# 42jaylonw/shifu

Measured on AMD Instinct MI355X. Metric: env-steps/sec (whole node), A1 12-dof 4096 envs/GPU, higher is better.
Workload: dtype f32

## Files before the change

### include/shifu_amd.h

```cpp
#ifndef SHIFU_AMD_H
#define SHIFU_AMD_H

#include <stdint.h>

#ifdef __cplusplus
extern "C" {
#endif

#define SHF_ABI_VERSION 22

#define SHF_MAX_BODIES 32
#define SHF_MAX_DOFS 32
#define SHF_MAX_POINTS 176
#define SHF_MAX_BOXES 4
#define SHF_MAX_SPHERES 8
#define SHF_MAX_CAPSULES 16
#define SHF_MAX_PAIRS 96
#define SHF_MAX_SELF_CONTACTS 8
#define SHF_MAX_ABOX 16
#define SHF_MAX_HARD_CONTACTS 16
#define SHF_MAX_LINK_CONTACTS 16

#define SHF_MAX_HULLS 8
#define SHF_HULL_MAX_VERTS 32
// ... 176 lines not shown
};
#define SHF_CONTACT_HIST_BINS 26

enum {
  SHF_REFRESH_DOF = 1,
  SHF_REFRESH_ROOT = 2,
  SHF_REFRESH_BODY = 4,
  SHF_REFRESH_CONTACT = 8,
  SHF_REFRESH_JACOBIAN = 16,
  SHF_REFRESH_ALL = 31
};

typedef struct ShfSim ShfSim;

const char* shf_last_error(void);
int shf_abi_version(void);

int shf_sim_create(const ShfSimParams* params, ShfSim** out);
int shf_sim_destroy(ShfSim* sim);
int shf_sim_set_terrain(ShfSim* sim, const ShfTerrain* terrain);
int shf_sim_set_articulation(ShfSim* sim, const ShfModel* model);
int shf_model_bounds(ShfModel* model);
int shf_model_pgs_supported(const ShfModel* model, int32_t nboxes);
int shf_sim_set_hulls(ShfSim* sim, const ShfHullSet* hulls);
int shf_convex_manifold(int32_t n, const float* pairs_dev, const ShfHull* hull_a_dev_or_null, float offset, int32_t lanes,
                        float* out_dev, void* stream);
#define SHF_CAP_TEST_SLOTS 88
int shf_cap_select_test(int32_t n, const float* gaps_dev, const uint8_t* flags_dev, const int32_t* kmax_dev, uint8_t* kept_dev, void* stream);
int shf_sim_set_scene_flags(ShfSim* sim, int32_t flags);
int shf_sim_add_box(ShfSim* sim, const ShfBoxDesc* box);
int shf_sim_finalize(ShfSim* sim, int32_t num_envs, int64_t env_id_offset);
int shf_sim_layout(const ShfSim* sim, int32_t id, int64_t shape[4], int32_t* ndim, int32_t* dtype);
int shf_sim_bind(ShfSim* sim, int32_t id, void* device_ptr);
int shf_sim_reset_all(ShfSim* sim, const float* default_root_dev , const float* default_dof_dev ,
                      const float* env_origins_dev , void* stream);
int shf_sim_set_group(ShfSim* sim, int32_t lanes);
enum { SHF_MAP_BODY = 0, SHF_MAP_CHAIN = 1, SHF_MAP_CHAIN_SPLIT = 2 };
int shf_sim_set_mapping(ShfSim* sim, int32_t mapping);

int shf_sim_step(ShfSim* sim, void* stream);
typedef struct ShfLaunchPlan {
  const char* kernel;
  int32_t grid, block;
  int64_t lds_bytes;
} ShfLaunchPlan;
int shf_sim_step_plan(const ShfSim* sim, ShfLaunchPlan* plan);
// ... 362 lines not shown
```

### shifu_amd/_lib.py

```python
import ctypes as C
import os

from . import _abi

_HERE = os.path.dirname(os.path.abspath(__file__))
_PATH = os.environ.get("SHIFU_AMD_LIB") or os.path.join(_HERE, "libshifu_amd.so")
_lib = None

vp, i32, i64 = C.c_void_p, C.c_int32, C.c_int64
_SIGS = {
    "shf_abi_version": ([], i32),
    "shf_sim_create": ([C.POINTER(_abi.ShfSimParams), C.POINTER(vp)], i32),
    "shf_sim_destroy": ([vp], i32),
    "shf_sim_set_terrain": ([vp, C.POINTER(_abi.ShfTerrain)], i32),
    "shf_sim_set_articulation": ([vp, C.POINTER(_abi.ShfModel)], i32),
    "shf_model_bounds": ([C.POINTER(_abi.ShfModel)], i32),
    "shf_model_pgs_supported": ([C.POINTER(_abi.ShfModel), i32], i32),
    "shf_abb_step_pgs_is_wide": ([vp], i32),
    "shf_sim_add_box": ([vp, C.POINTER(_abi.ShfBoxDesc)], i32),
    "shf_sim_set_hulls": ([vp, C.POINTER(_abi.ShfHullSet)], i32),
    "shf_sim_set_scene_flags": ([vp, i32], i32),
    "shf_convex_manifold": ([i32, vp, vp, C.c_float, i32, vp, vp], i32),
    "shf_cap_select_test": ([i32, vp, vp, vp, vp, vp], i32),
    "shf_sim_finalize": ([vp, i32, i64], i32),
    "shf_sim_set_group": ([vp, i32], i32),
    "shf_sim_set_mapping": ([vp, i32], i32),
    "shf_sim_layout": ([vp, i32, C.POINTER(i64), C.POINTER(i32), C.POINTER(i32)], i32),
    "shf_sim_bind": ([vp, i32, vp], i32),
    "shf_sim_reset_all": ([vp, vp, vp, vp, vp], i32),
    "shf_sim_step": ([vp, vp], i32),
    "shf_sim_step_plan": ([vp, C.POINTER(_abi.ShfLaunchPlan)], i32),
    "shf_sim_refresh": ([vp, i32, vp], i32),
    "shf_sim_dynamics": ([vp, vp, vp, vp], i32),
    "shf_sim_floating_dynamics": ([vp, vp, vp, vp, vp], i32),
    "shf_sim_set_dof_command": ([vp, i32, vp, vp], i32),
    "shf_sim_set_pos_target_indexed": ([vp, vp, vp, i32, vp], i32),
    "shf_sim_apply_body_force": ([vp, vp, vp], i32),
    "shf_sim_apply_body_force_at_pos": ([vp, vp, vp, vp], i32),
    "shf_sim_commit_root_indexed": ([vp, vp, vp, i32, vp], i32),
    "shf_sim_commit_root_all": ([vp, vp, vp], i32),
# ... 106 lines not shown
```

### shifu_amd/csrc/shf_a1_chain.hip

```cpp
#include <hip/hip_runtime.h>

#include "shf_chain.h"
#include "shf_chain_hard.h"

template <int G, bool TW, bool SELF = false>
__global__ __launch_bounds__(256, (G == 32 ? 2 : 1)) void k_a1_chain(A1Args A) { a1_chain_step_body<G, A1Chain, TW, SELF>(A); }

#ifndef SHF_WR_FUSED
#define SHF_WR_FUSED 8
#endif
#ifndef SHF_WR_HOOK
#define SHF_WR_HOOK 0
#endif
template <bool TW, bool SELF>
__global__ __launch_bounds__(256, 2) void k_a1_chain_pgs(A1Args A) { a1_chain_step_body<32, A1Chain, TW, SELF, true, 8, false, SHF_WR_FUSED>(A); }
template <bool TW, bool SELF>
__global__ __launch_bounds__(256, 2) void k_a1_chain_pgs16(A1Args A) { a1_chain_step_body<32, A1Chain, TW, SELF, true, 16>(A); }
template <bool TW, bool SELF>
__global__ __launch_bounds__(256, 2) void k_a1_chain_tgs(A1Args A) { a1_chain_step_body<32, A1Chain, TW, SELF, true, 8, true, SHF_WR_FUSED>(A); }
template <bool TW, bool SELF>
__global__ __launch_bounds__(256, 2) void k_a1_chain_tgs16(A1Args A) { a1_chain_step_body<32, A1Chain, TW, SELF, true, 16, true>(A); }
#define SHF_PICK4(K, warped, self) ((self) ? ((warped) ? reinterpret_cast<const void*>(K<true, true>) : reinterpret_cast<const void*>(K<false, true>)) \
                                           : ((warped) ? reinterpret_cast<const void*>(K<true, false>) : reinterpret_cast<const void*>(K<false, false>)))
const void* shf_a1_chain_pgs_kernel(bool warped, bool self, bool k16, bool tgs) {
  if (tgs) return k16 ? SHF_PICK4(k_a1_chain_tgs16, warped, self) : SHF_PICK4(k_a1_chain_tgs, warped, self);
  return k16 ? SHF_PICK4(k_a1_chain_pgs16, warped, self) : SHF_PICK4(k_a1_chain_pgs, warped, self);
}
int shf_a1_chain_pgs_max_contacts(void) { return 16; }

template <bool TW, bool SELF, int KC, bool TGS>
DEV void sim_step_chain_pgs_body(const SimArgs& A) {
  extern __shared__ __attribute__((aligned(16))) float smem[];
  typedef A1Chain CD;
  constexpr int G = 32, nb = CD::NB, nd = CD::ND, NR = (CD::NEV + G - 1) / G;
  const int es = threadIdx.x / G, l = threadIdx.x % G;
  const int e = blockIdx.x * (256 / G) + es;
  stage_block<CHAIN_MODEL_BYTES>(A.model, smem);
  __syncthreads();
  const ShfModel* m = reinterpret_cast<const ShfModel*>(smem);
  if (e >= A.n) return;
  ChainLds L = chain_lds_carve<CD>(smem + CHAIN_MODEL_WORDS + es * chain_lds_words<CD>(0, SELF));
  const float* dof = A.dof + (size_t)e * nd * 2;
  const float* root = A.root + (size_t)e * 13;
  for (int i = l; i < 2 * nd; i += G) L.dofb[(i >> 1) * DOF_STRIDE + (i & 1)] = dof[i];
  if (l < 13) L.root[l] = root[l];
  GROUP_SYNC();
  StepCtx C;
  C.m = m; C.sp = A.sp; C.terr.t = A.terr; C.terr.h = A.heights; C.scene = nullptr;
  C.dropped = env_dropped(A.dropped, A.sp, e);
  C.mscale = A.mscale ? A.mscale + (size_t)e * nb : nullptr;
  const float mu = A.friction ? A.friction[e] : 1.0f;
// ... 6 lines not shown
  chain_substep_hard<G, CD, TW, SELF, KC, TGS, (KC == 8 ? SHF_WR_HOOK : 0)>(C, L, l, X, LP, RL, A.body_force ? A.body_force + (size_t)e * nb * 3 : nullptr, mu, L.xch);
  if (l < nd) {
    A.dof[((size_t)e * nd + l) * 2] = X.q;
    A.dof[((size_t)e * nd + l) * 2 + 1] = X.qd;
  }
  if (l < 13) A.root[(size_t)e * 13 + l] = L.root[l];
  for (int i = l; i < 3 * nb; i += G) A.contact[(size_t)e * nb * 3 + i] = L.xch[i];
}
template <bool TW, bool SELF>
__global__ __launch_bounds__(256, 2) void k_sim_step_chain_pgs(SimArgs A) { sim_step_chain_pgs_body<TW, SELF, 8, false>(A); }
template <bool TW, bool SELF>
__global__ __launch_bounds__(256, 2) void k_sim_step_chain_pgs16(SimArgs A) { sim_step_chain_pgs_body<TW, SELF, 16, false>(A); }
template <bool TW, bool SELF>
__global__ __launch_bounds__(256, 2) void k_sim_step_chain_tgs(SimArgs A) { sim_step_chain_pgs_body<TW, SELF, 8, true>(A); }
template <bool TW, bool SELF>
__global__ __launch_bounds__(256, 2) void k_sim_step_chain_tgs16(SimArgs A) { sim_step_chain_pgs_body<TW, SELF, 16, true>(A); }
const void* shf_sim_step_chain_pgs_kernel(bool warped, bool self, bool k16, bool tgs) {
  if (tgs) return k16 ? SHF_PICK4(k_sim_step_chain_tgs16, warped, self) : SHF_PICK4(k_sim_step_chain_tgs, warped, self);
  return k16 ? SHF_PICK4(k_sim_step_chain_pgs16, warped, self) : SHF_PICK4(k_sim_step_chain_pgs, warped, self);
}
size_t shf_sim_step_chain_pgs_lds_bytes(bool self) { return ((size_t)CHAIN_MODEL_WORDS + 8 * (size_t)chain_lds_words<A1Chain>(0, self)) * 4; }

bool shf_a1_chain_matches(const ShfModel& m) { return A1Chain::matches(m); }
size_t shf_a1_chain_lds_bytes(int G, int nobs, bool self) {
  const int epb = 256 / G;
  return ((size_t)CHAIN_MODEL_WORDS + TASK_WORDS + STATS_LDS_WORDS + (size_t)epb * chain_lds_words<A1Chain>(SCR_OBS + nobs, self)) * 4;
}
const void* shf_a1_chain_kernel(int G, bool warped, bool self) {
  if (self) {
    if (G != 32) return nullptr;
    return warped ? reinterpret_cast<const void*>(k_a1_chain<32, true, true>) : reinterpret_cast<const void*>(k_a1_chain<32, false, true>);
  }
  switch (G) {
    case 16: return warped ? reinterpret_cast<const void*>(k_a1_chain<16, true>) : reinterpret_cast<const void*>(k_a1_chain<16, false>);
    case 32: return warped ? reinterpret_cast<const void*>(k_a1_chain<32, true>) : reinterpret_cast<const void*>(k_a1_chain<32, false>);
    default: return nullptr;
  }
}
#ifdef SHF_PHASE_CLOCK
int shf_a1_chain_phase_cycles(unsigned long long* out, int n, int reset) {
  unsigned long long h[48];
  if (hipMemcpyFromSymbol(h, HIP_SYMBOL(g_phase_cycles), sizeof h) != hipSuccess) return 1;
  for (int k = 0; k < n && k < 48; k++) out[k] = h[k];
  if (reset) {
    unsigned long long z[48] = {};
    if (hipMemcpyToSymbol(HIP_SYMBOL(g_phase_cycles), z, sizeof z) != hipSuccess) return 1;
  }
  return 0;
}
// ... 10 lines not shown
```

### shifu_amd/csrc/shf_api.hip

```cpp
#include <hip/hip_runtime.h>
#include <dlfcn.h>

#include <cstdio>
#include <cstring>
#include <initializer_list>
#include <map>
#include <mutex>
#include <type_traits>
#include <utility>
#include <vector>
#include <algorithm>
#include <cmath>
#include <string>

#include "shf_device.h"
#include "shf_task.h"
#include "shf_arm.h"
#include "shf_dyn.h"

static thread_local std::string g_err;
static int fail(const std::string& msg) { g_err = msg; return 1; }
int shf_set_error(const std::string& msg) { return fail(msg); }
#define HIP_OK(call)                                                              \
  do {                                                                            \
// ... 11 lines not shown
  int32_t n = 0;
  int64_t env_off = 0;
  bool finalized = false;
  bool force_armed = false;
  bool force_at_pos = false;
  void* t[SHF_T_COUNT] = {};
  int group = 64;
  int mapping = SHF_MAP_BODY;
  int mapping_split = 0;
  int chain_group = 16;
  ShfHullSet hulls;
  bool has_hulls = false;
  int scene_flags = 0;
};

struct ShfA1Task {
  ShfSim* sim;
  ShfA1TaskParams tp;
  void* t[SHF_A1_COUNT] = {};
  int stats_ring = 256;
};

bool shf_a1_chain_matches(const ShfModel& m);
size_t shf_a1_chain_lds_bytes(int G, int nobs, bool self);
const void* shf_a1_chain_kernel(int G, bool warped, bool self);
const void* shf_a1_chain_pgs_kernel(bool warped, bool self, bool k16, bool tgs);
int shf_a1_chain_pgs_max_contacts(void);
const void* shf_sim_step_chain_pgs_kernel(bool warped, bool self, bool k16, bool tgs);
size_t shf_sim_step_chain_pgs_lds_bytes(bool self);
#ifdef SHF_PHASE_CLOCK
int shf_a1_chain_phase_cycles(unsigned long long* out, int n, int reset);
int shf_a1_chain_phase_waves(unsigned long long* out, int reset);
#endif

extern "C" const char* shf_last_error(void) { return g_err.c_str(); }
extern "C" int shf_abi_version(void) { return SHF_ABI_VERSION; }


#define SHF_DEFINE_SMALL_KERNELS
#ifdef SHF_UNITY
#define SHF_DEFINE_A1_KERNELS
#endif
#include "shf_kernels.h"
#ifndef SHF_UNITY
#define SHF_KERNEL(...) extern template __global__ void __VA_ARGS__;
#include "shf_kernel_list.h"
#undef SHF_KERNEL
// ... 274 lines not shown
  A.scene = (const ShfScene*)s->t[SHF_T_SCENE];
  A.nboxes = s->nboxes;
  A.n = s->n;
  A.dof = (float*)s->t[internal ? SHF_T_SIM_DOF : SHF_T_DOF_STATE];
  A.root = (float*)s->t[internal ? SHF_T_SIM_ROOT : SHF_T_ROOT_STATE];
  A.actors = 1 + s->nboxes;
  A.effort = (const float*)s->t[SHF_T_EFFORT];
  A.pos_tgt = (const float*)s->t[SHF_T_POS_TARGET];
  A.vel_tgt = (const float*)s->t[SHF_T_VEL_TARGET];
  A.body_force = nullptr;
  A.body_force_pos = nullptr;
  A.friction = (const float*)s->t[SHF_T_FRICTION];
  A.mscale = (const float*)s->t[SHF_T_BODY_MASS_SCALE];
  A.contact = (float*)s->t[internal ? SHF_T_SIM_CONTACT : SHF_T_CONTACT];
  A.dropped = (int32_t*)s->t[SHF_T_DROPPED];
  A.hulls = (s->model.nhull > 0 && s->model.link_collide != 0) ? (const ShfHullSet*)s->t[SHF_T_HULLS] : nullptr;
  if (s->t[SHF_T_CONTACT_HIST]) {
    A.dropped = (int32_t*)s->t[SHF_T_CONTACT_HIST];
    A.sp.max_contacts = (A.sp.max_contacts & 0xff) | SHF_HIST_FLAG;
  }
  return A;
}

static int lds_fits(size_t lds) {
  return lds > 160 * 1024 ? fail("kernel needs " + std::to_string(lds) + " B of LDS per block, the CU has 160 KiB") : 0;
}
static int grant_lds(const void* fn, size_t lds) {
  if (int r = lds_fits(lds)) return r;
  if (lds > 48 * 1024) {
    static std::mutex mu;
    static std::map<std::pair<int, const void*>, size_t> granted;
    int dev = 0;
    HIP_OK(hipGetDevice(&dev));
    std::lock_guard<std::mutex> lock(mu);
    size_t& have = granted[{dev, fn}];
    if (have < lds) {
      HIP_OK(hipFuncSetAttribute(fn, hipFuncAttributeMaxDynamicSharedMemorySize, (int)lds));
      have = lds;
    }
  }
  return 0;
}
template <typename K, typename... Args>
static int launch(K kernel, dim3 grid, dim3 block, size_t lds, void* stream, Args... args) {
  if (int r = grant_lds(reinterpret_cast<const void*>(kernel), lds)) return r;
  hipLaunchKernelGGL(kernel, grid, block, lds, (hipStream_t)stream, args...);
  HIP_OK(hipGetLastError());
  return 0;
// ... 345 lines not shown
  A.push = (float*)task->t[SHF_A1_PUSH]; A.origins = (float*)task->t[SHF_A1_ORIGINS];
  A.levels = (int64_t*)task->t[SHF_A1_LEVELS]; A.types = (const int64_t*)task->t[SHF_A1_TYPES];
  A.torigins = (const float*)task->t[SHF_A1_TORIGINS];
  A.reset_count = (int32_t*)task->t[SHF_A1_RESET_COUNT];
  A.done_sums = (float*)task->t[SHF_A1_DONE_SUMS];
  A.body_state = (float*)s->t[SHF_T_BODY_STATE];
  A.stats.acc = (unsigned long long*)task->t[SHF_A1_STATS_ACC];
  A.stats.out = (float*)task->t[SHF_A1_STATS];
  A.stats.ring = task->stats_ring;
  A.stats.out_cols = 16;
  return 0;
}

static int a1_step_plan(const ShfA1Task* task, Plan& P) {
  const ShfSim* s = task->sim;
  const int nobs = 12 + 2 * s->model.nd + s->model.nd * task->tp.num_history + task->tp.num_height_points;
  const int g = s->group, n = s->n;
  const bool self = sim_self(s), warped = s->terr.warped != 0;
  if (s->sp.solver != SHF_SOLVER_COMPLIANT) {
    if (s->mapping != SHF_MAP_CHAIN || s->chain_group != 32 || !shf_a1_chain_matches(s->model))
      return fail("shf_a1_step: ShfSimParams.solver = SHF_SOLVER_PGS runs on the chain mapping at 32 lanes per env (shf_sim_set_mapping)");
    if (s->sp.max_contacts > shf_a1_chain_pgs_max_contacts()) return fail("shf_a1_step: the fused A1 step's solve holds at most 16 constraints per env (ShfSimParams.max_contacts)");
    if (s->sp.pos_iters < 1) return fail("shf_a1_step: ShfSimParams.pos_iters must be >= 1 with SHF_SOLVER_PGS");
    return set_plan(P, shf_a1_chain_pgs_kernel(warped, self, s->sp.max_contacts > HCK, s->sp.solver == SHF_SOLVER_TGS), n, 8, 256, shf_a1_chain_lds_bytes(32, nobs, self));
  }
  if (s->mapping == SHF_MAP_CHAIN) {
    if (!shf_a1_chain_matches(s->model)) return fail("shf_a1_step: the articulation does not fit the chain mapping");
    const void* fn = shf_a1_chain_kernel(s->chain_group, warped, self);
    if (!fn) return fail(self ? "shf_a1_step: the chain mapping with self-collision runs at 32 lanes per env"
                              : "shf_a1_step: the chain mapping runs at 16 or 32 lanes per env");
    return set_plan(P, fn, n, 256 / s->chain_group, 256, shf_a1_chain_lds_bytes(s->chain_group, nobs, self));
  }
  if (warped && g == 64)
    return fail("shf_a1_step: a trimesh terrain needs 16 or 32 lanes per env (the 128-VGPR instantiation has no room for it)");
  if (self && g == 64) return fail("shf_a1_step: self-collision needs 16 or 32 lanes per env (no register room in the 128-VGPR instantiation)");
  const bool a1 = A1Dims::matches(s->model);
  if (a1 && g == 16) return fail("shf_a1_step: A1 has 17 bodies, the lane group must be 32 or 64");
  const void* fn;
  if (!a1) fn = self ? (g == 32 ? KFN(k_a1_step_self<32, DynDims>) : KFN(k_a1_step_self<16, DynDims>)) : PICK_LANES(g, k_a1_step, DynDims);
  else if (self) fn = warped ? KFN(k_a1_step_self<32, A1Dims>) : KFN(k_a1_step_self_a1_g32);
  else fn = g == 64 ? KFN(k_a1_step<64, A1Dims>) : warped ? KFN(k_a1_step<32, A1Dims>) : KFN(k_a1_step_a1_g32);
  return set_plan(P, fn, n, 256 / g, 256, sim_lds_bytes(s, g, TASK_WORDS + STATS_LDS_WORDS, SCR_OBS + nobs));
}
extern "C" int shf_a1_step_plan(const ShfA1Task* task, ShfLaunchPlan* out) {
  if (!task) return fail("shf_a1_step: null task");
  if (!out) return fail("shf_a1_step_plan: null argument");
  Plan P;
  return export_plan(a1_step_plan(task, P), P, out);
}
static int a1_step_launch(ShfA1Task* task, const float* raw_actions_dev, void* stream) {
  A1Args A;
  if (int r = a1_args(task, raw_actions_dev, "shf_a1_step", A)) return r;
  Plan P;
  if (int r = a1_step_plan(task, P)) return r;
// ... 200 lines not shown
```

### shifu_amd/csrc/shf_chain.h

```cpp
#pragma once
#include "shf_task.h"
#include "shf_link.h"

template <int NCH_, int NLK_, int NP_, int NEV_>
struct ChainDims {
  static constexpr int NCH = NCH_, NLK = NLK_, NB = 1 + NCH_ * (NLK_ + 1), ND = NCH_ * NLK_, NPC = NP_;
  static constexpr int NEV = NEV_;
  static constexpr int MAXPT = 9;
  static_assert(NEV_ >= NP_ && NEV_ <= 128, "evaluation slots: two 64-bit ballot words");
  DEV static constexpr int body(int c, int k) { return 1 + c * (NLK_ + 1) + k; }
  static bool matches(const ShfModel& m) {
    if (m.nb != NB || m.nd != ND || m.np != NPC || m.fixed_base || m.jtype[0] != SHF_JOINT_ROOT) return false;
    if (m.child_count[0] != NCH || m.nlevels != NLK) return false;
    if ((m.neval > 0 ? m.neval : m.np) != NEV) return false;
    int occupied = 0;
    for (int s = 0; s < NEV; s++) {
      const int i = m.pt_eval[s];
      if (i == -1) continue;
      if (i < 0 || i >= NPC || m.pt_slot[i] != s) return false;
      occupied++;
    }
    if (occupied != NPC) return false;
    for (int b = 0; b < NB; b++) {
      const int n = m.pt_count[b], i0 = m.pt_start[b];
// ... 23 lines not shown
};
typedef ChainDims<4, 3, 76, 88> A1Chain;

#define JREC_STRIDE 16
#define JREC_QD 9
#define JREC_T0 12
#define JREC_DE 13
#define JREC_S 0
#define JREC_C 6
#define CHAIN_MODEL_BYTES ((int)offsetof(ShfModel, link_collide))
#define CHAIN_MODEL_WORDS ((CHAIN_MODEL_BYTES / 4 + 3) & ~3)
static_assert(CHAIN_MODEL_BYTES % 16 == 0, "stage_block copies 16-byte words");
template <class CD>
__host__ __device__ inline int chain_lds_words(int min_tail, bool self = false) {
  int tail = (CD::NPC + (self ? SHF_MAX_SELF_CONTACTS : 0)) * PT_STRIDE;
  if (tail < min_tail) tail = min_tail;
  const int w = CD::NB * POSE_STRIDE + ((CD::NB * 6 + 3) & ~3) + (CD::ND + 1) * XCH_STRIDE + CD::ND * JREC_STRIDE +
                ((CD::ND * DOF_STRIDE + 3) & ~3) + root_words(1) + tail;
  return (w + 3) & ~3;
}
struct ChainLds : EnvLds {
  float* jrec;
  float* xroot;
};
template <class CD>
DEV ChainLds chain_lds_carve(float* base) {
  static_assert(CD::ND * XCH_STRIDE >= 3 * CD::NB, "the exchange slots double as the contact-force staging");
  ChainLds L;
  L.pose = base;
  L.acc = L.pose + CD::NB * POSE_STRIDE;
  L.xch = L.acc + ((CD::NB * 6 + 3) & ~3);
  L.xroot = L.xch + CD::ND * XCH_STRIDE;
  L.jrec = L.xroot + XCH_STRIDE;
  L.dofb = L.jrec + CD::ND * JREC_STRIDE;
  L.root = L.dofb + ((CD::ND * DOF_STRIDE + 3) & ~3);
  L.pt = L.root + root_words(1);
  return L;
}

DEV void chain_ext_force(const float* F, const float* com, const float* Rw, const float* p, float* pA) {
  if (F[0] == 0.0f && F[1] == 0.0f && F[2] == 0.0f) return;
  float cw[3], t[3];
  mv3(Rw, com, cw);
#pragma unroll
  for (int k = 0; k < 3; k++) cw[k] += p[k];
  cross3(cw, F, t);
// ... 43 lines not shown
    const int s = l + k * G;
    const int e = s < nev ? m->pt_eval[s] : -1;
    const int i = e < 0 ? 0 : e;
    P.idx[k] = e;
    P.body[k] = m->pt_body[i];
    P.rad[k] = m->pt_radius[i];
    P.thr[k] = (offset + P.rad[k]) * 1.01f + 1e-6f;
#pragma unroll
    for (int j = 0; j < 3; j++) P.pos[k][j] = m->pt_pos[i][j];
  }
}

DEV void terrain_height_gradient(const TerrainDev& T, float x, float y, float* h, float* gxo, float* gyo) {
  if (T.t.rows == 0) { *h = 0.0f; *gxo = 0.0f; *gyo = 0.0f; return; }
  float inv = 1.0f / T.t.hscale;
  float fx = (x + T.t.border) * inv, fy = (y + T.t.border) * inv;
  float fi = rclampf(floorf(fx), 0.0f, (float)(T.t.rows - 2)), fj = rclampf(floorf(fy), 0.0f, (float)(T.t.cols - 2));
  int i = (int)fi, j = (int)fj;
  float u = rclampf(fx - fi, 0.0f, 1.0f), v = rclampf(fy - fj, 0.0f, 1.0f);
  float vs = T.t.vscale;
  const int16_t* row0 = T.h + (size_t)i * T.t.cols + j;
  const int16_t* row1 = row0 + T.t.cols;
  float h00 = (float)row0[0] * vs, h10 = (float)row1[0] * vs, h01 = (float)row0[1] * vs, h11 = (float)row1[1] * vs;
  const bool lo = u + v <= 1.0f;
  float gx = (lo ? h10 : h11) - (lo ? h00 : h01);
  float gy = (lo ? h01 : h11) - (lo ? h00 : h10);
  *h = fmaf(lo ? v : 1.0f - v, lo ? gy : -gy, fmaf(lo ? u : 1.0f - u, lo ? gx : -gx, lo ? h00 : h11));
  *gxo = gx * inv; *gyo = gy * inv;
}
DEV void terrain_normal_from_gradient(const TerrainDev& T, float gx, float gy, float* n) {
  if (T.t.rows == 0) { n[0] = 0.0f; n[1] = 0.0f; n[2] = 1.0f; return; }
  const float nz = rsqrt_spec(fmaf(gy, gy, fmaf(gx, gx, 1.0f)));
  n[0] = -gx * nz; n[1] = -gy * nz; n[2] = nz;
}

struct SlotBits {
  unsigned long long w[2];
  DEV bool test(int s) const { return ((s < 64 ? w[0] >> s : w[1] >> (s - 64)) & 1ull) != 0ull; }
  DEV unsigned field(int s0, int n) const {
    const unsigned long long ww = s0 < 64 ? w[0] : w[1];
    return (unsigned)(ww >> (s0 & 63)) & ((1u << n) - 1u);
  }
};
template <int MAXPT>
struct SlotList {
  unsigned long long list;
// ... 521 lines not shown
  GROUP_SYNC();
  for (int b = l; b < NB; b += G) {
    const float* pb = L.pose + b * POSE_STRIDE;
    float Rw[9], pp[3], v[6], t[3], q[4];
#pragma unroll
    for (int k = 0; k < 9; k++) Rw[k] = pb[k];
#pragma unroll
    for (int k = 0; k < 3; k++) pp[k] = pb[9 + k];
#pragma unroll
    for (int k = 0; k < 6; k++) v[k] = pb[12 + k];
    float* o = stage + 13 * b;
#pragma unroll
    for (int k = 0; k < 3; k++) o[k] = L.root[k] + pp[k];
    mat_to_quat(Rw, q);
#pragma unroll
    for (int k = 0; k < 4; k++) o[3 + k] = q[k];
    cross3(v, pp, t);
#pragma unroll
    for (int k = 0; k < 3; k++) { o[7 + k] = v[3 + k] + t[k]; o[10 + k] = v[k]; }
  }
  GROUP_SYNC();
}

template <int G, class CD, bool TW, bool SELF, int KC, bool TGS, int WR>
DEV void chain_substep_hard(const StepCtx& C, const ChainLds& L, int l, DofLane& X, const ChainPoints<(CD::NEV + G - 1) / G>& P,
                            const RowLane& RL, const float* fext, float mu_shape, float* contact_out);
template <int G, class CD, bool TW, bool SELF = false, bool HARD = false, int KC = 8, bool TGS = false, int WR = 0>
DEV void a1_chain_step_body(const A1Args& A) {
  extern __shared__ __attribute__((aligned(16))) float smem[];
  constexpr int NLK = CD::NLK, nb = CD::NB, nd = CD::ND, NR = (CD::NEV + G - 1) / G;
  PHASE_BEGIN();
  float* stats_lds = smem + CHAIN_MODEL_WORDS + TASK_WORDS;
  stats_block_init(stats_lds);
  const int epb = 256 / G, es = threadIdx.x / G, l = threadIdx.x % G;
  const int e = blockIdx.x * epb + es;
  const int n = A.S.n;
  const unsigned long long stats_req = stats_step_request(A.stats);
  const uint64_t seed = A.tp->seed;
  __builtin_amdgcn_sched_barrier(0);
  constexpr int NW = (2 * nd + G - 1) / G;
  float pre_dof[NW], pre_root = 0.0f, pre_act = 0.0f;
#pragma unroll
  for (int k = 0; k < NW; k++) pre_dof[k] = 0.0f;
  static_assert(G >= 13 && G > nd, "one root word and one action per lane");
  const bool given = A.raw_actions != nullptr;
  if (e < n) {
#pragma unroll
    for (int k = 0; k < NW; k++)
      if (l + k * G < 2 * nd) pre_dof[k] = A.S.dof[(size_t)e * nd * 2 + l + k * G];
    if (l < 13) pre_root = A.S.root[(size_t)e * 13 + l];
    if (l < nd && given) pre_act = A.raw_actions[(size_t)e * nd + l];
  }
  StagedBlock<(int)sizeof(ShfA1TaskParams)> tp_words;
  StagedBlock<CHAIN_MODEL_BYTES> model_words;
  tp_words.load(A.tp);
  model_words.load(A.S.model);
  const unsigned long long stats_step = stats_step_take(stats_req);
  constexpr bool POSTFIX = !(HARD && !TGS);
  const unsigned stats_row_index = POSTFIX ? stats_slot(A.stats, stats_step) : 0u;
  if (e < n && l < nd && !given) pre_act = random_action(seed, A.env_off + e, stats_step, l);
#pragma unroll
  for (int k = 0; k < NW; k++) asm volatile("" : "+v"(pre_dof[k]));
  asm volatile("" : "+v"(pre_root), "+v"(pre_act));
  tp_words.pin();
  model_words.pin();
  tp_words.store(smem + CHAIN_MODEL_WORDS);
  model_words.store(smem);
  __syncthreads();
  PHASE_MARK(23);
  const ShfModel* m = reinterpret_cast<const ShfModel*>(smem);
  const ShfA1TaskParams& tp = *reinterpret_cast<const ShfA1TaskParams*>(smem + CHAIN_MODEL_WORDS);
  if (e >= n) return;
  const int H = tp.num_history, P = tp.num_height_points;
  const int nobs = 12 + 2 * nd + nd * H + P;
  const int env_words = chain_lds_words<CD>(SCR_OBS + nobs, SELF);
  ChainLds L = chain_lds_carve<CD>(smem + CHAIN_MODEL_WORDS + TASK_WORDS + STATS_LDS_WORDS + es * env_words);
  float* scr = L.pt;

#pragma unroll
  for (int k = 0; k < NW; k++) {
    const int i = l + k * G;
    if (i < 2 * nd) L.dofb[(i >> 1) * DOF_STRIDE + (i & 1)] = pre_dof[k];
  }
  if (l < 13) L.root[l] = pre_root;
  float act = 0.0f;
  if (l < nd) {
    act = rclampf(pre_act * tp.action_scale, -tp.clip_actions, tp.clip_actions);
    A.actions[(size_t)e * nd + l] = act;
  }
  GROUP_SYNC();

  if (l == 0) {
    const float gv[3] = {0.0f, 0.0f, -1.0f};
    float pg[3], blv[3], bav[3];
    quat_rotate_inverse(L.root + 3, L.root + 7, blv);
    quat_rotate_inverse(L.root + 3, L.root + 10, bav);
    quat_rotate_inverse(L.root + 3, gv, pg);
    float* o = A.base_vel + (size_t)e * 9;
#pragma unroll
    for (int k = 0; k < 3; k++) { o[k] = blv[k]; o[3 + k] = bav[k]; o[6 + k] = pg[k]; }
  }

  StepCtx C;
  C.m = m; C.sp = A.S.sp; C.terr.t = A.S.terr; C.terr.h = A.S.heights; C.scene = nullptr;
  if constexpr (HARD) C.dropped = env_dropped(A.S.dropped, A.S.sp, e);
  C.mscale = A.S.mscale ? A.S.mscale + (size_t)e * nb : nullptr;
  const float mu = A.S.friction[e];
  const int nsub = tp.decimation + (tp.extra_substep ? 1 : 0);
  const int dl = l < nd ? l : 0;
  DofLane X = {L.dofb[dl * DOF_STRIDE], L.dofb[dl * DOF_STRIDE + 1], 0.0f};
  const float pg_ = tp.p_gain[dl], dg_ = tp.d_gain[dl], q0_ = tp.default_dof_pos[dl], lim_ = m->effort[dl];
  ChainPoints<NR> LP;
  if constexpr (!(HARD && WR > 0)) chain_points_load<G>(m, CD::NEV, l, HARD ? C.sp.contact_offset + C.sp.rest_offset : C.sp.contact_offset, LP);
  const int lb = G >= 32 ? (l & 15) : l;
  const int mb = lb < nd ? CD::body(lb / NLK, lb % NLK) : 0;
  const SlotList<CD::MAXPT> mine = slot_list_load<CD::MAXPT>(m, m->pt_start[mb], (lb <= nd && l < 32) ? m->pt_count[mb] : 0);
  const RowLane RL = row_lane_load<CD>(l);
  PHASE_MARK(11);
  for (int it = 0; it < nsub; it++) {
    if (it < tp.decimation) {
      const float t = pg_ * (act + q0_ - X.q) - dg_ * X.qd;
      X.tau = rclampf(t, -lim_, lim_);
    }
    if constexpr (HARD)
      chain_substep_hard<G, CD, TW, SELF, KC, TGS, WR>(C, L, l, X, LP, RL, (it == tp.decimation) ? A.push + (size_t)e * nb * 3 : nullptr, mu,
                                    (it == nsub - 1) ? L.xch : nullptr);
    else
      chain_substep<G, CD, TW, SELF>(C, L, l, X, LP, mine, RL, (it == tp.decimation) ? A.push + (size_t)e * nb * 3 : nullptr, mu,
                                     (it == nsub - 1) ? L.xch : nullptr);
  }
  PHASE_RESET();
  const A1Args AE = a1_args_again();
  if (l < nd) {
    float* D = L.dofb + l * DOF_STRIDE;
    D[0] = X.q; D[1] = X.qd; D[5] = X.tau;
    AE.torques[(size_t)e * nd + l] = X.tau;
    scr[SCR_ACT + l] = act;
  }
  for (int i = l; i < 3 * nb; i += G) AE.S.contact[(size_t)e * nb * 3 + i] = L.xch[i];
  for (int i = l; i < nd * H; i += G) scr[SCR_HIST + i] = AE.history[(size_t)e * nd * H + i];
  PHASE_MARK(12);
  chain_body_states<G, CD>(m, L, l, X, scr + SCR_BODY);
  for (int i = l; i < 13 * nb; i += G) AE.body_state[(size_t)e * nb * 13 + i] = scr[SCR_BODY + i];
  PHASE_MARK(13);
  if constexpr (POSTFIX) a1_post_step<G, nd, nb>(AE, m, tp, L, scr, e, l, stats_lds, stats_step, stats_row_index);
  else a1_post_step<G>(AE, m, tp, L, scr, e, l, stats_lds, stats_step);
}
```

### shifu_amd/csrc/shf_chain_hard.h

```cpp
#pragma once
#include "shf_chain.h"

#define UF_STRIDE 8
template <class CD, int KC>
struct HardTail {
  static constexpr int HC = 0, W = KC * HC_STRIDE, NEVP = (CD::NEV + 3) & ~3;
  static constexpr bool PACKED = KC > 8;
  static constexpr int WS = PACKED ? 9 : 10;
  static constexpr int NBLK = PACKED ? KC * (KC + 1) / 2 : KC * KC;
  static constexpr int NB0 = PACKED ? (CD::NPC * PT_STRIDE - W) / 9 : NBLK;
  static constexpr int UF = W, PHI = W, END = W + NB0 * WS;
  static constexpr int SPARE = CD::NB * POSE_STRIDE + ((CD::NB * 6 + 3) & ~3) + CD::ND * XCH_STRIDE;
  static_assert(NEVP + SHF_MAX_SELF_CONTACTS <= NB0 * WS && CD::ND * UF_STRIDE <= NB0 * WS, "the gap list / U, 1/D fit the response matrix's place");
  static_assert(!PACKED || (NBLK - NB0) * 9 <= SPARE, "the rest of the packed response matrix fits the pose / rate / exchange slots");
  static_assert(KC <= 16 && (W % 2) == 0, "owner lanes, 16-bit constraint masks; 8-byte aligned blocks");
};
template <class CD, int KC>
DEV float* hard_wblock(const ChainLds& L, float* tail, int i, int j) {
  typedef HardTail<CD, KC> T;
  if constexpr (T::PACKED) {
    const int b = ((j * (j + 1)) >> 1) + i;
    return b < T::NB0 ? tail + T::W + b * 9 : L.pose + (b - T::NB0) * 9;
  } else {
    return tail + T::W + (j * KC + i) * T::WS;
// ... 315 lines not shown
  for (int k = 0; k < NR; k++) {
    const int q = hard_gap_key(ph[k]);
    key[k] = cand[k] ? (keep ? -q : q) : NONE;
  }
  if constexpr (SELF) {
    const int q = hard_gap_key(sph);
    skey = scand ? (keep ? -q : q) : NONE;
  }
  int n = keep ? 0 : excess;
  while (__ballot(n > 0) != 0ull) {
    hard_cap_extract<G, NR, SELF, true>(l, lane0, n > 0, key, skey);
    n--;
  }
  n = keep ? kmax : 0;
  while (__ballot(n > 0) != 0ull) {
    hard_cap_extract<G, NR, SELF, false>(l, lane0, n > 0, key, skey);
    n--;
  }
#pragma unroll
  for (int k = 0; k < NR; k++) cand[k] = cand[k] && ((key[k] == NONE) == keep);
  if constexpr (SELF) scand = scand && ((skey == NONE) == keep);
}

template <int G, class CD, bool TW, bool SELF, int KC, bool TGS, int WR>
DEV void chain_substep_hard(const StepCtx& C, const ChainLds& L, int l, DofLane& X, const ChainPoints<(CD::NEV + G - 1) / G>& PIN,
                            const RowLane& RL, const float* fext, float mu_shape, float* contact_out) {
  static_assert(G == 32, "the velocity-level solve is written for two envs per wavefront");
  constexpr int NCH = CD::NCH, NLK = CD::NLK, NB = CD::NB, ND = CD::ND, NR = (CD::NEV + G - 1) / G;
  typedef HardTail<CD, KC> T;
  static_assert(T::END <= CD::NPC * PT_STRIDE, "the solve's LDS fits the contact-slot region");
  static_assert((KC == 8 || KC == 16) && KC <= G / 2 + 8 && ND < 16, "owner lanes; a lane per column of the response matrix, in one or two passes");
  static_assert(WR >= 0 && WR <= KC && (WR == 0 || !T::PACKED), "the register row is the KC = 8 layout's");
  constexpr bool PIPE = WR > 0 && !SELF;
  constexpr bool SPLIT4 = WR > 0;
  constexpr bool CAPREG = !(SELF && (KC > 8 || (WR > 0 && TGS)));
  constexpr bool DROPATOM = WR > 0 && !TGS;
  const ShfModel* m = C.m;
  const float dt = C.sp.dt, idt = 1.0f / dt;
  const float gon = (float)m->gravity_on;
  const float g[3] = {C.sp.gravity[0] * gon, C.sp.gravity[1] * gon, C.sp.gravity[2] * gon};
  float* tail = L.pt;
  const int lb = l & 15;
  const int half = (l >> 4) & 1;
  const bool isdof = l < ND, isroot = l == ND;
  const bool ischain = (l & 7) == 0 && (l >> 3) < NCH;
  const int ci = l >> 3;
  const bool isbody = lb <= ND;
// ... 85 lines not shown
    }
    float* o = (islink ? L.xch + lb * XCH_STRIDE : L.xroot);
    if (half == 0) {
#pragma unroll
      for (int j = 0; j < 11; j++) o[j] = IA[j];
    } else {
#pragma unroll
      for (int j = 11; j < 21; j++) o[j] = IA[j];
#pragma unroll
      for (int j = 0; j < 6; j++) o[21 + j] = pA[j];
    }
  }
  PHASE_MARK(2);

  const float rest = C.sp.rest_offset, offs = C.sp.contact_offset + rest;
  const float mu = 0.5f * (mu_shape + C.terr.t.friction);
  const int kmax = hard_kmax_of(C.sp, KC);
  SlotBits act = {{0ull, 0ull}};
  int K;
  {
    float r[NR][3], nn[NR][3], ph[NR], gx[NR], gy[NR], dz[NR];
    bool near[NR], cand[NR];
    const float nzmin = TW ? 0.0f : C.terr.t.nz_min;
#pragma unroll
    for (int k = 0; k < NR; k++) {
      const float* pb = L.pose + P.body[k] * POSE_STRIDE;
      float Rb[9], h = 0.0f;
#pragma unroll
      for (int j = 0; j < 9; j++) Rb[j] = pb[j];
      mv3(Rb, P.pos[k], r[k]);
#pragma unroll
      for (int j = 0; j < 3; j++) r[k][j] += pb[9 + j];
      if constexpr (TW) {
        gx[k] = 0.0f; gy[k] = 0.0f; dz[k] = 0.0f;
        near[k] = P.idx[k] >= 0;
      } else {
        terrain_height_gradient(C.terr, L.root[0] + r[k][0], L.root[1] + r[k][1], &h, &gx[k], &gy[k]);
        dz[k] = L.root[2] + r[k][2] - h;
        near[k] = P.idx[k] >= 0 && !(dz[k] * nzmin >= P.thr[k]);
      }
    }
#pragma unroll
    for (int k = 0; k < NR; k++) {
      cand[k] = false; ph[k] = 0.0f;
      if (__ballot(near[k]) == 0ull) continue;
      if (near[k]) {
        float phi;
        if constexpr (TW) {
          float h;
          terrain_query<true>(C.terr, L.root[0] + r[k][0], L.root[1] + r[k][1], &h, nn[k]);
          phi = fmaf(L.root[2] + r[k][2] - h, nn[k][2], -P.rad[k]);
        } else {
          terrain_normal_from_gradient(C.terr, gx[k], gy[k], nn[k]);
          phi = fmaf(dz[k], nn[k][2], -P.rad[k]);
        }
        if (phi < offs) {
          cand[k] = true;
          ph[k] = phi - rest;
#pragma unroll
          for (int j = 0; j < 3; j++) r[k][j] = fmaf(-P.rad[k], nn[k][j], r[k][j]);
        }
      }
      const unsigned long long bits = (__ballot(cand[k]) >> lane0) & ((1ull << G) - 1ull);
// ... 602 lines not shown
```

### shifu_amd/csrc/shf_device.h

```cpp
#pragma once
#include <hip/hip_runtime.h>
#include <stdint.h>

#include "../../include/shifu_amd.h"

#define DEV __device__ __forceinline__

#define GROUP_SYNC()                                         \
  do {                                                       \
    __builtin_amdgcn_fence(__ATOMIC_RELEASE, "workgroup");   \
    __builtin_amdgcn_wave_barrier();                         \
    __builtin_amdgcn_fence(__ATOMIC_ACQUIRE, "workgroup");   \
  } while (0)

#ifdef SHF_PHASE_CLOCK
#define PHASE_NK 48
#define PHASE_NW 2048
__device__ unsigned long long g_phase_cycles[PHASE_NK];
__device__ unsigned long long g_phase_wave[PHASE_NW][PHASE_NK];
#define PHASE_BEGIN() unsigned long long _pc = clock64()
#define PHASE_MARK(k)                                                                    \
  do {                                                                                   \
    const unsigned long long _now = clock64();                                           \
    if (blockIdx.x == 0 && threadIdx.x == 0) g_phase_cycles[k] += _now - _pc;            \
    const unsigned _pw = blockIdx.x * (blockDim.x >> 6) + (threadIdx.x >> 6);            \
    if ((threadIdx.x & 63u) == 0u && _pw < PHASE_NW) atomicAdd(&g_phase_wave[_pw][k], _now - _pc);   \
    _pc = clock64();                                                                     \
  } while (0)
#define PHASE_RESET() _pc = clock64()
#define PHASE_PARAM , unsigned long long& _pc
#define PHASE_PASS , _pc
#define PHASE_BEGIN_T() unsigned long long _pct = clock64()
#define PHASE_MARK_T(k, tid)                                                             \
  do {                                                                                   \
    const unsigned long long _now = clock64();                                           \
    if (blockIdx.x == 0 && (int)threadIdx.x == (tid)) g_phase_cycles[k] += _now - _pct;  \
    _pct = clock64();                                                                    \
  } while (0)
#else
#define PHASE_BEGIN_T() do {} while (0)
#define PHASE_MARK_T(k, tid) do {} while (0)
#define PHASE_BEGIN() do {} while (0)
#define PHASE_MARK(k) do {} while (0)
#define PHASE_RESET() do {} while (0)
#define PHASE_PARAM
#define PHASE_PASS
#endif

DEV float rcp_spec(float x) {
  float y = __uint_as_float(0x7EF311C7u - __float_as_uint(x));
#pragma unroll
  for (int k = 0; k < 3; k++) { const float e = fmaf(-x, y, 1.0f); y = fmaf(y, e, y); }
  return y;
}
DEV float rsqrt_spec(float x) {
  float y = __uint_as_float(0x5F375A86u - (__float_as_uint(x) >> 1));
  const float hx = 0.5f * x;
#pragma unroll
  for (int k = 0; k < 3; k++) { const float t = y * y; const float w = fmaf(-hx, t, 1.5f); y = y * w; }
  return y;
}

// ... 1197 lines not shown
```

Before: 27.91 million.

## Stage a per-env 16x16 height-field patch in LDS for PGS contact queries

Before the substep loop, each env loads a 16x16 window of the int16 height field around its root into LDS, at half a row per lane. Per-substep terrain height and gradient lookups then read samples from that LDS window and fall back to global memory only for points outside it. This targets the cost of scattered global height-field reads in the contact detection phase of the fused A1 PGS kernel. It adds LDS per env, checked against two blocks per CU, plus a prologue load, and it only applies to the non-warped, non-self, 8-contact PGS path.

```diff
diff --git a/include/shifu_amd.h b/include/shifu_amd.h
--- a/include/shifu_amd.h
+++ b/include/shifu_amd.h
@@ -222,6 +222,7 @@
 int shf_sim_set_articulation(ShfSim* sim, const ShfModel* model);
 int shf_model_bounds(ShfModel* model);
 int shf_model_pgs_supported(const ShfModel* model, int32_t nboxes);
+int shf_terrain_patch_origin(const ShfTerrain* terrain, float x, float y, int32_t* i0, int32_t* j0, int32_t* side);
 int shf_sim_set_hulls(ShfSim* sim, const ShfHullSet* hulls);
 int shf_convex_manifold(int32_t n, const float* pairs_dev, const ShfHull* hull_a_dev_or_null, float offset, int32_t lanes,
                         float* out_dev, void* stream);
diff --git a/shifu_amd/_lib.py b/shifu_amd/_lib.py
--- a/shifu_amd/_lib.py
+++ b/shifu_amd/_lib.py
@@ -16,6 +16,7 @@
     "shf_sim_set_articulation": ([vp, C.POINTER(_abi.ShfModel)], i32),
     "shf_model_bounds": ([C.POINTER(_abi.ShfModel)], i32),
     "shf_model_pgs_supported": ([C.POINTER(_abi.ShfModel), i32], i32),
+    "shf_terrain_patch_origin": ([C.POINTER(_abi.ShfTerrain), C.c_float, C.c_float, C.POINTER(i32), C.POINTER(i32), C.POINTER(i32)], i32),
     "shf_abb_step_pgs_is_wide": ([vp], i32),
     "shf_sim_add_box": ([vp, C.POINTER(_abi.ShfBoxDesc)], i32),
     "shf_sim_set_hulls": ([vp, C.POINTER(_abi.ShfHullSet)], i32),
diff --git a/shifu_amd/csrc/shf_a1_chain.hip b/shifu_amd/csrc/shf_a1_chain.hip
--- a/shifu_amd/csrc/shf_a1_chain.hip
+++ b/shifu_amd/csrc/shf_a1_chain.hip
@@ -1,4 +1,6 @@
 #include <hip/hip_runtime.h>
+
+#include <string>
 
 #include "shf_chain.h"
 #include "shf_chain_hard.h"
@@ -12,12 +14,18 @@
 #ifndef SHF_WR_HOOK
 #define SHF_WR_HOOK 0
 #endif
+#ifndef SHF_PATCH_TGS
+#define SHF_PATCH_TGS 0
+#endif
+#ifndef SHF_PATCH_PGS
+#define SHF_PATCH_PGS 1
+#endif
 template <bool TW, bool SELF>
-__global__ __launch_bounds__(256, 2) void k_a1_chain_pgs(A1Args A) { a1_chain_step_body<32, A1Chain, TW, SELF, true, 8, false, SHF_WR_FUSED>(A); }
+__global__ __launch_bounds__(256, 2) void k_a1_chain_pgs(A1Args A) { a1_chain_step_body<32, A1Chain, TW, SELF, true, 8, false, SHF_WR_FUSED, SHF_PATCH_PGS && !TW && !SELF>(A); }
 template <bool TW, bool SELF>
 __global__ __launch_bounds__(256, 2) void k_a1_chain_pgs16(A1Args A) { a1_chain_step_body<32, A1Chain, TW, SELF, true, 16>(A); }
 template <bool TW, bool SELF>
-__global__ __launch_bounds__(256, 2) void k_a1_chain_tgs(A1Args A) { a1_chain_step_body<32, A1Chain, TW, SELF, true, 8, true, SHF_WR_FUSED>(A); }
+__global__ __launch_bounds__(256, 2) void k_a1_chain_tgs(A1Args A) { a1_chain_step_body<32, A1Chain, TW, SELF, true, 8, true, SHF_WR_FUSED, SHF_PATCH_TGS && !TW && !SELF>(A); }
 template <bool TW, bool SELF>
 __global__ __launch_bounds__(256, 2) void k_a1_chain_tgs16(A1Args A) { a1_chain_step_body<32, A1Chain, TW, SELF, true, 16, true>(A); }
 #define SHF_PICK4(K, warped, self) ((self) ? ((warped) ? reinterpret_cast<const void*>(K<true, true>) : reinterpret_cast<const void*>(K<false, true>)) \
@@ -27,6 +35,15 @@
   return k16 ? SHF_PICK4(k_a1_chain_pgs16, warped, self) : SHF_PICK4(k_a1_chain_pgs, warped, self);
 }
 int shf_a1_chain_pgs_max_contacts(void) { return 16; }
+bool shf_a1_chain_pgs_patch(bool warped, bool self, bool k16, bool tgs) { return !warped && !self && !k16 && (tgs ? SHF_PATCH_TGS : SHF_PATCH_PGS) != 0; }
+int shf_set_error(const std::string& msg);
+extern "C" int shf_terrain_patch_origin(const ShfTerrain* terrain, float x, float y, int32_t* i0, int32_t* j0, int32_t* side) {
+  if (!terrain || !i0 || !j0 || !side) return shf_set_error("shf_terrain_patch_origin: null argument");
+  int a, b;
+  terrain_patch_origin(x, y, terrain->border, terrain->hscale, terrain->rows, terrain->cols, &a, &b);
+  *i0 = a == TERRAIN_PATCH_NONE ? -1 : a; *j0 = b == TERRAIN_PATCH_NONE ? -1 : b; *side = TERRAIN_PATCH_S;
+  return 0;
+}
 
 template <bool TW, bool SELF, int KC, bool TGS>
 DEV void sim_step_chain_pgs_body(const SimArgs& A) {
@@ -79,9 +96,9 @@
 size_t shf_sim_step_chain_pgs_lds_bytes(bool self) { return ((size_t)CHAIN_MODEL_WORDS + 8 * (size_t)chain_lds_words<A1Chain>(0, self)) * 4; }
 
 bool shf_a1_chain_matches(const ShfModel& m) { return A1Chain::matches(m); }
-size_t shf_a1_chain_lds_bytes(int G, int nobs, bool self) {
+size_t shf_a1_chain_lds_bytes(int G, int nobs, bool self, bool patch) {
   const int epb = 256 / G;
-  return ((size_t)CHAIN_MODEL_WORDS + TASK_WORDS + STATS_LDS_WORDS + (size_t)epb * chain_lds_words<A1Chain>(SCR_OBS + nobs, self)) * 4;
+  return ((size_t)CHAIN_MODEL_WORDS + TASK_WORDS + STATS_LDS_WORDS + (size_t)epb * (chain_lds_words<A1Chain>(SCR_OBS + nobs, self) + (patch ? TERRAIN_PATCH_WORDS : 0))) * 4;
 }
 const void* shf_a1_chain_kernel(int G, bool warped, bool self) {
   if (self) {
diff --git a/shifu_amd/csrc/shf_api.hip b/shifu_amd/csrc/shf_api.hip
--- a/shifu_amd/csrc/shf_api.hip
+++ b/shifu_amd/csrc/shf_api.hip
@@ -57,7 +57,8 @@
 };
 
 bool shf_a1_chain_matches(const ShfModel& m);
-size_t shf_a1_chain_lds_bytes(int G, int nobs, bool self);
+size_t shf_a1_chain_lds_bytes(int G, int nobs, bool self, bool patch);
+bool shf_a1_chain_pgs_patch(bool warped, bool self, bool k16, bool tgs);
 const void* shf_a1_chain_kernel(int G, bool warped, bool self);
 const void* shf_a1_chain_pgs_kernel(bool warped, bool self, bool k16, bool tgs);
 int shf_a1_chain_pgs_max_contacts(void);
@@ -378,8 +379,9 @@
   return A;
 }
 
-static int lds_fits(size_t lds) {
-  return lds > 160 * 1024 ? fail("kernel needs " + std::to_string(lds) + " B of LDS per block, the CU has 160 KiB") : 0;
+static int lds_fits(size_t lds, int blocks_per_cu = 1) {
+  return lds * blocks_per_cu > 160 * 1024 ? fail("kernel needs " + std::to_string(lds) + " B of LDS per block" +
+                                                 (blocks_per_cu > 1 ? " at " + std::to_string(blocks_per_cu) + " blocks per CU" : std::string()) + ", the CU has 160 KiB") : 0;
 }
 static int grant_lds(const void* fn, size_t lds) {
   if (int r = lds_fits(lds)) return r;
@@ -771,14 +773,18 @@
       return fail("shf_a1_step: ShfSimParams.solver = SHF_SOLVER_PGS runs on the chain mapping at 32 lanes per env (shf_sim_set_mapping)");
     if (s->sp.max_contacts > shf_a1_chain_pgs_max_contacts()) return fail("shf_a1_step: the fused A1 step's solve holds at most 16 constraints per env (ShfSimParams.max_contacts)");
     if (s->sp.pos_iters < 1) return fail("shf_a1_step: ShfSimParams.pos_iters must be >= 1 with SHF_SOLVER_PGS");
-    return set_plan(P, shf_a1_chain_pgs_kernel(warped, self, s->sp.max_contacts > HCK, s->sp.solver == SHF_SOLVER_TGS), n, 8, 256, shf_a1_chain_lds_bytes(32, nobs, self));
+    const bool k16 = s->sp.max_contacts > HCK, tgs = s->sp.solver == SHF_SOLVER_TGS;
+    const bool patch = shf_a1_chain_pgs_patch(warped, self, k16, tgs);
+    const size_t lds = shf_a1_chain_lds_bytes(32, nobs, self, patch);
+    if (patch) if (int r = lds_fits(lds, 2)) return r;
+    return set_plan(P, shf_a1_chain_pgs_kernel(warped, self, k16, tgs), n, 8, 256, lds);
   }
   if (s->mapping == SHF_MAP_CHAIN) {
     if (!shf_a1_chain_matches(s->model)) return fail("shf_a1_step: the articulation does not fit the chain mapping");
     const void* fn = shf_a1_chain_kernel(s->chain_group, warped, self);
     if (!fn) return fail(self ? "shf_a1_step: the chain mapping with self-collision runs at 32 lanes per env"
                               : "shf_a1_step: the chain mapping runs at 16 or 32 lanes per env");
-    return set_plan(P, fn, n, 256 / s->chain_group, 256, shf_a1_chain_lds_bytes(s->chain_group, nobs, self));
+    return set_plan(P, fn, n, 256 / s->chain_group, 256, shf_a1_chain_lds_bytes(s->chain_group, nobs, self, false));
   }
   if (warped && g == 64)
     return fail("shf_a1_step: a trimesh terrain needs 16 or 32 lanes per env (the 128-VGPR instantiation has no room for it)");
diff --git a/shifu_amd/csrc/shf_chain.h b/shifu_amd/csrc/shf_chain.h
--- a/shifu_amd/csrc/shf_chain.h
+++ b/shifu_amd/csrc/shf_chain.h
@@ -69,6 +69,7 @@
 struct ChainLds : EnvLds {
   float* jrec;
   float* xroot;
+  const int16_t* patch = nullptr;
 };
 template <class CD>
 DEV ChainLds chain_lds_carve(float* base) {
@@ -158,6 +159,43 @@
   const int16_t* row0 = T.h + (size_t)i * T.t.cols + j;
   const int16_t* row1 = row0 + T.t.cols;
   float h00 = (float)row0[0] * vs, h10 = (float)row1[0] * vs, h01 = (float)row0[1] * vs, h11 = (float)row1[1] * vs;
+  const bool lo = u + v <= 1.0f;
+  float gx = (lo ? h10 : h11) - (lo ? h00 : h01);
+  float gy = (lo ? h01 : h11) - (lo ? h00 : h10);
+  *h = fmaf(lo ? v : 1.0f - v, lo ? gy : -gy, fmaf(lo ? u : 1.0f - u, lo ? gx : -gx, lo ? h00 : h11));
+  *gxo = gx * inv; *gyo = gy * inv;
+}
+#define TERRAIN_PATCH_S 16
+#define TERRAIN_PATCH_WORDS (TERRAIN_PATCH_S * TERRAIN_PATCH_S / 2)
+#define TERRAIN_PATCH_NONE 0x40000000
+__host__ __device__ inline void terrain_patch_origin(float x, float y, float border, float hscale, int rows, int cols, int* i0, int* j0) {
+  constexpr int S = TERRAIN_PATCH_S;
+  if (rows < S || cols < S) { *i0 = TERRAIN_PATCH_NONE; *j0 = TERRAIN_PATCH_NONE; return; }
+  const float inv = 1.0f / hscale;
+  const float fx = (x + border) * inv, fy = (y + border) * inv;
+  const int ci = fx >= 0.0f ? (fx < (float)(rows - 2) ? (int)fx : rows - 2) : 0;
+  const int cj = fy >= 0.0f ? (fy < (float)(cols - 2) ? (int)fy : cols - 2) : 0;
+  int a = ci - (S / 2 - 1), b = cj - (S / 2 - 1);
+  a = a < 0 ? 0 : a; b = b < 0 ? 0 : b;
+  *i0 = a > rows - S ? rows - S : a;
+  *j0 = b > cols - S ? cols - S : b;
+}
+DEV void terrain_cell(const TerrainDev& T, float x, float y, int* io, int* jo, float* uo, float* vo) {
+  float inv = 1.0f / T.t.hscale;
+  float fx = (x + T.t.border) * inv, fy = (y + T.t.border) * inv;
+  float fi = rclampf(floorf(fx), 0.0f, (float)(T.t.rows - 2)), fj = rclampf(floorf(fy), 0.0f, (float)(T.t.cols - 2));
+  *io = (int)fi; *jo = (int)fj;
+  *uo = rclampf(fx - fi, 0.0f, 1.0f); *vo = rclampf(fy - fj, 0.0f, 1.0f);
+}
+DEV void terrain_samples_global(const TerrainDev& T, int i, int j, int16_t* s) {
+  const int16_t* row0 = T.h + (size_t)i * T.t.cols + j;
+  const int16_t* row1 = row0 + T.t.cols;
+  s[0] = row0[0]; s[1] = row1[0]; s[2] = row0[1]; s[3] = row1[1];
+}
+DEV void terrain_height_gradient_from(const TerrainDev& T, const int16_t* s, float u, float v, float* h, float* gxo, float* gyo) {
+  float inv = 1.0f / T.t.hscale;
+  float vs = T.t.vscale;
+  float h00 = (float)s[0] * vs, h10 = (float)s[1] * vs, h01 = (float)s[2] * vs, h11 = (float)s[3] * vs;
   const bool lo = u + v <= 1.0f;
   float gx = (lo ? h10 : h11) - (lo ? h00 : h01);
   float gy = (lo ? h01 : h11) - (lo ? h00 : h10);
@@ -725,11 +763,12 @@
   GROUP_SYNC();
 }
 
-template <int G, class CD, bool TW, bool SELF, int KC, bool TGS, int WR>
+template <int G, class CD, bool TW, bool SELF, int KC, bool TGS, int WR, bool PATCH = false>
 DEV void chain_substep_hard(const StepCtx& C, const ChainLds& L, int l, DofLane& X, const ChainPoints<(CD::NEV + G - 1) / G>& P,
                             const RowLane& RL, const float* fext, float mu_shape, float* contact_out);
-template <int G, class CD, bool TW, bool SELF = false, bool HARD = false, int KC = 8, bool TGS = false, int WR = 0>
+template <int G, class CD, bool TW, bool SELF = false, bool HARD = false, int KC = 8, bool TGS = false, int WR = 0, bool PATCH = false>
 DEV void a1_chain_step_body(const A1Args& A) {
+  static_assert(!PATCH || (HARD && !TW && G == 32), "the patch is phase P's of the velocity-level solve on the height field");
   extern __shared__ __attribute__((aligned(16))) float smem[];
   constexpr int NLK = CD::NLK, nb = CD::NB, nd = CD::ND, NR = (CD::NEV + G - 1) / G;
   PHASE_BEGIN();
@@ -774,6 +813,19 @@
   const ShfModel* m = reinterpret_cast<const ShfModel*>(smem);
   const ShfA1TaskParams& tp = *reinterpret_cast<const ShfA1TaskParams*>(smem + CHAIN_MODEL_WORDS);
   if (e >= n) return;
+  int patch_i0 = TERRAIN_PATCH_NONE, patch_j0 = TERRAIN_PATCH_NONE;
+  uint4 patch_w;
+  if constexpr (PATCH) {
+    static_assert(TERRAIN_PATCH_S == 16 && G == 32, "half a row of the window per lane");
+    const float rx = __shfl(pre_root, 0, G), ry = __shfl(pre_root, 1, G);
+    const int16_t* src = reinterpret_cast<const int16_t*>(A.tp);
+    if (A.S.terr.rows != 0) {
+      terrain_patch_origin(rx, ry, A.S.terr.border, A.S.terr.hscale, A.S.terr.rows, A.S.terr.cols, &patch_i0, &patch_j0);
+      if (patch_i0 != TERRAIN_PATCH_NONE) src = A.S.heights + (size_t)(patch_i0 + (l >> 1)) * A.S.terr.cols + patch_j0 + 8 * (l & 1);
+    }
+    __builtin_memcpy(&patch_w, src, sizeof patch_w);
+    __builtin_amdgcn_sched_barrier(0);
+  }
   const int H = tp.num_history, P = tp.num_height_points;
   const int nobs = 12 + 2 * nd + nd * H + P;
   const int env_words = chain_lds_words<CD>(SCR_OBS + nobs, SELF);
@@ -786,6 +838,10 @@
     if (i < 2 * nd) L.dofb[(i >> 1) * DOF_STRIDE + (i & 1)] = pre_dof[k];
   }
   if (l < 13) L.root[l] = pre_root;
+  if constexpr (PATCH) {
+    if (l == 13) L.root[13] = __int_as_float(patch_i0);
+    if (l == 14) L.root[14] = __int_as_float(patch_j0);
+  }
   float act = 0.0f;
   if (l < nd) {
     act = rclampf(pre_act * tp.action_scale, -tp.clip_actions, tp.clip_actions);
@@ -819,6 +875,12 @@
   const int mb = lb < nd ? CD::body(lb / NLK, lb % NLK) : 0;
   const SlotList<CD::MAXPT> mine = slot_list_load<CD::MAXPT>(m, m->pt_start[mb], (lb <= nd && l < 32) ? m->pt_count[mb] : 0);
   const RowLane RL = row_lane_load<CD>(l);
+  if constexpr (PATCH) {
+    __builtin_amdgcn_sched_barrier(0);
+    int16_t* pw = reinterpret_cast<int16_t*>(smem + CHAIN_MODEL_WORDS + TASK_WORDS + STATS_LDS_WORDS + epb * env_words + es * TERRAIN_PATCH_WORDS);
+    L.patch = pw;
+    *reinterpret_cast<uint4*>(pw + 8 * l) = patch_w;
+  }
   PHASE_MARK(11);
   for (int it = 0; it < nsub; it++) {
     if (it < tp.decimation) {
@@ -826,7 +888,7 @@
       X.tau = rclampf(t, -lim_, lim_);
     }
     if constexpr (HARD)
-      chain_substep_hard<G, CD, TW, SELF, KC, TGS, WR>(C, L, l, X, LP, RL, (it == tp.decimation) ? A.push + (size_t)e * nb * 3 : nullptr, mu,
+      chain_substep_hard<G, CD, TW, SELF, KC, TGS, WR, PATCH>(C, L, l, X, LP, RL, (it == tp.decimation) ? A.push + (size_t)e * nb * 3 : nullptr, mu,
                                     (it == nsub - 1) ? L.xch : nullptr);
     else
       chain_substep<G, CD, TW, SELF>(C, L, l, X, LP, mine, RL, (it == tp.decimation) ? A.push + (size_t)e * nb * 3 : nullptr, mu,
diff --git a/shifu_amd/csrc/shf_chain_hard.h b/shifu_amd/csrc/shf_chain_hard.h
--- a/shifu_amd/csrc/shf_chain_hard.h
+++ b/shifu_amd/csrc/shf_chain_hard.h
@@ -361,7 +361,7 @@
   if constexpr (SELF) scand = scand && ((skey == NONE) == keep);
 }
 
-template <int G, class CD, bool TW, bool SELF, int KC, bool TGS, int WR>
+template <int G, class CD, bool TW, bool SELF, int KC, bool TGS, int WR, bool PATCH>
 DEV void chain_substep_hard(const StepCtx& C, const ChainLds& L, int l, DofLane& X, const ChainPoints<(CD::NEV + G - 1) / G>& PIN,
                             const RowLane& RL, const float* fext, float mu_shape, float* contact_out) {
   static_assert(G == 32, "the velocity-level solve is written for two envs per wavefront");
@@ -493,6 +493,53 @@
     float r[NR][3], nn[NR][3], ph[NR], gx[NR], gy[NR], dz[NR];
     bool near[NR], cand[NR];
     const float nzmin = TW ? 0.0f : C.terr.t.nz_min;
+    if constexpr (PATCH) {
+      static_assert(!TW, "the patch holds height-field samples");
+      constexpr int S = TERRAIN_PATCH_S;
+      float hh[NR];
+#pragma unroll
+      for (int k = 0; k < NR; k++) {
+        const float* pb = L.pose + P.body[k] * POSE_STRIDE;
+        float Rb[9];
+#pragma unroll
+        for (int j = 0; j < 9; j++) Rb[j] = pb[j];
+        mv3(Rb, P.pos[k], r[k]);
+#pragma unroll
+        for (int j = 0; j < 3; j++) r[k][j] += pb[9 + j];
+        hh[k] = 0.0f; gx[k] = 0.0f; gy[k] = 0.0f;
+      }
+      if (C.terr.t.rows != 0) {
+        const float rx = L.root[0], ry = L.root[1];
+        const int i0 = __float_as_int(L.root[13]), j0 = __float_as_int(L.root[14]);
+        typedef __attribute__((address_space(3))) int16_t lds_i16;
+        const lds_i16* patch = (const lds_i16*)L.patch;
+        int ci[NR], cj[NR];
+        float cu[NR], cv[NR];
+        bool in[NR];
+        int16_t smp[NR][4];
+#pragma unroll
+        for (int k = 0; k < NR; k++) {
+          terrain_cell(C.terr, rx + r[k][0], ry + r[k][1], &ci[k], &cj[k], &cu[k], &cv[k]);
+          in[k] = (unsigned)(ci[k] - i0) <= (unsigned)(S - 2) && (unsigned)(cj[k] - j0) <= (unsigned)(S - 2);
+          const lds_i16* ps = patch + (in[k] ? (ci[k] - i0) * S + (cj[k] - j0) : 0);
+          smp[k][0] = ps[0]; smp[k][1] = ps[S]; smp[k][2] = ps[1]; smp[k][3] = ps[S + 1];
+        }
+#pragma unroll
+        for (int k = 0; k < NR; k++) {
+          if (__ballot(!in[k]) != 0ull) {
+            if (!in[k]) terrain_samples_global(C.terr, ci[k], cj[k], smp[k]);
+            PATCH_COUNT_FALLBACK(__popcll(__ballot(!in[k])));
+          }
+          PATCH_COUNT_ROWS(__popcll(__ballot(true)));
+          terrain_height_gradient_from(C.terr, smp[k], cu[k], cv[k], &hh[k], &gx[k], &gy[k]);
+        }
+      }
+#pragma unroll
+      for (int k = 0; k < NR; k++) {
+        dz[k] = L.root[2] + r[k][2] - hh[k];
+        near[k] = P.idx[k] >= 0 && !(dz[k] * nzmin >= P.thr[k]);
+      }
+    } else {
 #pragma unroll
     for (int k = 0; k < NR; k++) {
       const float* pb = L.pose + P.body[k] * POSE_STRIDE;
@@ -510,6 +557,7 @@
         dz[k] = L.root[2] + r[k][2] - h;
         near[k] = P.idx[k] >= 0 && !(dz[k] * nzmin >= P.thr[k]);
       }
+    }
     }
 #pragma unroll
     for (int k = 0; k < NR; k++) {
diff --git a/shifu_amd/csrc/shf_device.h b/shifu_amd/csrc/shf_device.h
--- a/shifu_amd/csrc/shf_device.h
+++ b/shifu_amd/csrc/shf_device.h
@@ -37,7 +37,21 @@
     if (blockIdx.x == 0 && (int)threadIdx.x == (tid)) g_phase_cycles[k] += _now - _pct;  \
     _pct = clock64();                                                                    \
   } while (0)
+#ifdef SHF_PATCH_COUNT
+#define PHASE_COUNT(k, n)                                                                \
+  do {                                                                                   \
+    const unsigned long long _n = (unsigned long long)(n), _b = __ballot(true);          \
+    if ((int)(threadIdx.x & 63u) == __ffsll(_b) - 1) atomicAdd(&g_phase_cycles[k], _n);  \
+  } while (0)
+#define PATCH_COUNT_FALLBACK(n) PHASE_COUNT(36, n)
+#define PATCH_COUNT_ROWS(n) PHASE_COUNT(37, n)
 #else
+#define PATCH_COUNT_FALLBACK(n) do {} while (0)
+#define PATCH_COUNT_ROWS(n) do {} while (0)
+#endif
+#else
+#define PATCH_COUNT_FALLBACK(n) do {} while (0)
+#define PATCH_COUNT_ROWS(n) do {} while (0)
 #define PHASE_BEGIN_T() do {} while (0)
 #define PHASE_MARK_T(k, tid) do {} while (0)
 #define PHASE_BEGIN() do {} while (0)
```

Result: no change. 27.90 million (median of 2 runs) (-0.0%).
